# starlingonearth/MASt3R-SLAM-Quality-dualTSDF

Hardware: AMD Instinct MI355X
Metric: SLAM frames/sec (infer+match+TSDF+GN) @512x384 (higher is better)
Workload: dtype bf16

## Files before the change

### include/mslam_hip.h

```cpp
#ifndef MSLAM_HIP_H
#define MSLAM_HIP_H

#include <stddef.h>
#include <stdint.h>

#ifdef __cplusplus
extern "C" {
#endif

#define MSLAM_OK 0
#define MSLAM_EINVAL (-1)
#define MSLAM_EHIP (-2)
#define MSLAM_ENOMEM (-3)
#define MSLAM_ENODEV (-4)

const char* mslam_last_error(void);
int mslam_abi_version(void);
int mslam_device_check(void);


int mslam_iter_proj(const float* rays_img_with_grad, const float* pts_3d_norm,
                    const float* p_init, float* p_new, uint8_t* converged, int b, int h, int w,
                    int n, int max_iter, float lambda_init, float cost_thresh, void* stream);

// ... 39 lines not shown
int mslam_gn_compact(const float* Xs, const float* Cs, const int64_t* idx_ii2jj, const uint8_t* valid_match,
                     const float* Q, int num_poses, int num_points, int num_edges, int edge_begin,
                     int edge_count, float C_thresh, float Q_thresh, void* workspace, size_t workspace_bytes,
                     void* stream);
int mslam_gn_compact_at(const float* Xs, const float* Cs, const int64_t* idx_ii2jj, const uint8_t* valid_match,
                        const float* Q, int num_poses, int num_points, int num_edges, int edge_begin, int edge_count,
                        int slot_begin, int range_count, float C_thresh, float Q_thresh, void* workspace,
                        size_t workspace_bytes, void* stream);
int mslam_gn_accumulate(int kind, const float* Twc, const float* K, int num_poses, int num_points,
                        int num_edges, int edge_begin, int edge_count, float sigma_a, float sigma_b,
                        int height, int width, int pixel_border, float z_eps, float* Hs, float* gs,
                        void* workspace, size_t workspace_bytes, void* stream);
int mslam_gn_solve_retract(const float* Hs, const float* gs, int num_poses, int num_edges,
                           int num_points, float* Twc, float* dx, float delta_thresh, void* workspace,
                           size_t workspace_bytes, void* stream);
int mslam_gn_status(int* status4, int num_poses, int num_edges, int num_points, void* workspace,
                    size_t workspace_bytes, void* stream);

int mslam_sim3_act(const float* T, const float* X, float* Y, int num_poses, long long pts_per_pose,
                   int broadcast_pose, void* stream);
int mslam_sim3_op(int op, const float* A, const float* B, float* out, int n, int bcast_a, int bcast_b,
                  void* stream);

size_t mslam_tsdf_table_bytes(uint64_t capacity);
int mslam_tsdf_table_init(void* table, size_t table_bytes, uint64_t capacity, void* stream);

size_t mslam_tsdf_integrate_workspace_bytes(int n_points, double voxel_size, double trunc, double step_scale);
int mslam_tsdf_integrate(void* table, uint64_t capacity, const float* points_world, const double* conf,
                         const float* cam_origin, int n_points, double voxel_size, double trunc,
                         double max_weight, double step_scale, int shard_id, int num_shards,
// ... 244 lines not shown
```

### mast3r-slam-quality-dualtsdf_amd/csrc/gn.hip

```cpp
#include "common.h"
#include "sim3.h"

namespace mslam {

constexpr int kAcc = 35;
constexpr int kEdgeConst = 16;
constexpr int kPlanes = 8;
constexpr int kTile = 64;

struct GnState {
  int done;
  int iters;
  int chol_fail;
  float last_norm;
};

__device__ __forceinline__ int64_t ij_val(const int64_t* ii, const int64_t* jj, int E, int k) {
  return k < E ? ii[k] : jj[k - E];
}

__global__ __launch_bounds__(256) void gn_first_kernel(const int64_t* __restrict__ ii,
                                                       const int64_t* __restrict__ jj, int E,
                                                       int* __restrict__ first) {
  const int k = blockIdx.x * 256 + threadIdx.x;
// ... 25 lines not shown
  if (st->done) return;
  const int e = blockIdx.x * blockDim.x + threadIdx.x;
  if (e >= E) return;
  const Sim3f Ti = sim3_load(Twc + 8 * ii_edge[e]);
  const Sim3f Tj = sim3_load(Twc + 8 * jj_edge[e]);
  const Sim3f Tij = sim3_rel(Ti, Tj);
  float R[9];
  quat_to_mat(Tij.q, R);
  float* c = econst + (size_t)e * kEdgeConst;
#pragma unroll
  for (int k = 0; k < 9; k++) c[k] = Tij.s * R[k];
  c[9] = Tij.t[0]; c[10] = Tij.t[1]; c[11] = Tij.t[2];
  c[12] = c[13] = c[14] = c[15] = 0.0f;
}

__global__ __launch_bounds__(256) void gn_compact_kernel(
    const float* __restrict__ Xs, const float* __restrict__ Cs, const int* __restrict__ ii_edge,
    const int* __restrict__ jj_edge, const int64_t* __restrict__ idx_ii2jj,
    const uint8_t* __restrict__ valid_match, const float* __restrict__ Q, int num_points, int chunk_len,
    float C_thresh, float Q_thresh, float* __restrict__ stream, int* __restrict__ counts, int S, int slot_begin) {
  const int e = blockIdx.x / S, chunk = blockIdx.x - e * S;
  const int ix = ii_edge[e], jx = jj_edge[e];
  const float* __restrict__ Xi_base = Xs + (size_t)ix * num_points * 3;
  const float* __restrict__ Xj_base = Xs + (size_t)jx * num_points * 3;
  const float* __restrict__ Ci_base = Cs + (size_t)ix * num_points;
  const float* __restrict__ Cj_base = Cs + (size_t)jx * num_points;
  const int64_t* __restrict__ idx_e = idx_ii2jj + (size_t)e * num_points;
  const uint8_t* __restrict__ vm_e = valid_match + (size_t)e * num_points;
  const float* __restrict__ Q_e = Q + (size_t)e * num_points;
  float* __restrict__ slot = stream + ((size_t)(slot_begin + e) * S + chunk) * (size_t)chunk_len * kPlanes;
  __shared__ int wave_cnt[4];
  const int lane = threadIdx.x & 63, wid = threadIdx.x >> 6;
  const int k_begin = chunk * chunk_len;
  const int k_end = min(k_begin + chunk_len, num_points);
  int base = 0;
  for (int k0 = k_begin; k0 < k_end; k0 += 256) {
    const int k = k0 + (int)threadIdx.x;
    bool valid = false;
    long long ind = 0;
    float q = 0.0f;
    if (k < k_end) {
      const bool vm = vm_e[k] != 0;
      ind = vm ? idx_e[k] : 0;
      q = Q_e[k];
      const float ci = Ci_base[ind], cj = Cj_base[k];
      valid = vm & (q > Q_thresh) & (ci > C_thresh) & (cj > C_thresh);
    }
    const unsigned long long m = __ballot(valid);
    if (lane == 0) wave_cnt[wid] = __popcll(m);
    __syncthreads();
    int off = base;
    for (int w = 0; w < wid; w++) off += wave_cnt[w];
    const int total = wave_cnt[0] + wave_cnt[1] + wave_cnt[2] + wave_cnt[3];
    if (valid) {
      const int pos = off + __popcll(m & ((1ull << lane) - 1ull));
      slot[0 * (size_t)chunk_len + pos] = Xi_base[ind * 3 + 0];
      slot[1 * (size_t)chunk_len + pos] = Xi_base[ind * 3 + 1];
      slot[2 * (size_t)chunk_len + pos] = Xi_base[ind * 3 + 2];
      slot[3 * (size_t)chunk_len + pos] = Xj_base[(size_t)k * 3 + 0];
      slot[4 * (size_t)chunk_len + pos] = Xj_base[(size_t)k * 3 + 1];
      slot[5 * (size_t)chunk_len + pos] = Xj_base[(size_t)k * 3 + 2];
      slot[6 * (size_t)chunk_len + pos] = sqrtf(q);
      slot[7 * (size_t)chunk_len + pos] = __int_as_float((int)ind);
    }
    base += total;
    __syncthreads();
  }
  if (threadIdx.x == 0) counts[(slot_begin + e) * S + chunk] = base;
}

__device__ __forceinline__ float fast_rcp(float x) { return __builtin_amdgcn_rcpf(x); }
__device__ __forceinline__ float fast_rsq(float x) { return __builtin_amdgcn_rsqf(x); }

__device__ __forceinline__ float huber_w(float r) {
  return fminf(1.0f, 1.345f * fast_rcp(fabsf(r)));
}

template <unsigned NZ>
__device__ __forceinline__ void accum_row(float (&acc)[kAcc], const float (&x)[7], float w, float err) {
  const float we = w * err;
  int l = 0;
#pragma unroll
  for (int n = 0; n < 7; n++) {
// ... 100 lines not shown
    {
      const float x[7] = {1.0f, 0.0f, 0.0f, 0.0f, p2, -p1, p0};
      accum_row<0b1110001>(acc, x, w0, e0);
    }
    {
      const float x[7] = {0.0f, 1.0f, 0.0f, -p2, 0.0f, p0, p1};
      accum_row<0b1101010>(acc, x, w1, e1);
    }
    {
      const float x[7] = {0.0f, 0.0f, 1.0f, p1, -p0, 0.0f, p2};
      accum_row<0b1011100>(acc, x, w2, e2);
    }
  }
}

template <int KIND>
__global__ __launch_bounds__(256) void gn_accum_kernel(const GnState* __restrict__ st,
                                                       const float* __restrict__ econst,
                                                       const float* __restrict__ stream,
                                                       const int* __restrict__ counts, int chunk_len,
                                                       GnParams P, float* __restrict__ partial, int S) {
  if (st->done) return;
  const int e = blockIdx.x / S, chunk = blockIdx.x - e * S;
  const float* cc = econst + (size_t)e * kEdgeConst;
  const EdgeConst c = {cc[0], cc[1], cc[2], cc[3], cc[4], cc[5], cc[6], cc[7], cc[8], cc[9], cc[10], cc[11]};
  const float* __restrict__ slot = stream + ((size_t)e * S + chunk) * (size_t)chunk_len * kPlanes;
  const int n = counts[e * S + chunk];

  float acc[kAcc];
#pragma unroll
  for (int l = 0; l < kAcc; l++) acc[l] = 0.0f;

  const int n4 = n & ~3;
  for (int k = (int)threadIdx.x * 4; k < n4; k += 1024) {
    float f[kPlanes][4];
#pragma unroll
    for (int p = 0; p < kPlanes; p++) {
      if (p < (KIND == 1 ? 8 : 7)) {
        const float4 v = *reinterpret_cast<const float4*>(slot + (size_t)p * chunk_len + k);
        f[p][0] = v.x; f[p][1] = v.y; f[p][2] = v.z; f[p][3] = v.w;
      } else {
        f[p][0] = f[p][1] = f[p][2] = f[p][3] = 0.0f;
// ... 558 lines not shown
  float* econst;
  float* Hs;
  float* gs;
  double* Haug;
  double* Ldiag;
  double* xs;
  int* tmin32;
  int* counts;
  float* partial;
  float* stream;
  int S, chunk_len, np, ld, nb;
  size_t bytes_fixed;
  size_t bytes;
};

static GnWorkspace gn_carve(void* base, int P, int E, int HW, int local_edges) {
  GnWorkspace w;
  const int N = P > 1 ? P - 1 : 0;
  const int n = N * 7;
  w.np = (int)align_up((size_t)(n > 0 ? n : 1), kTile);
  w.ld = w.np;
  w.nb = 32;
  int S = E > 0 ? (1024 + E - 1) / E : 1;
  const int s_cap = HW / (256 * 16) > 0 ? HW / (256 * 16) : 1;
  if (S > s_cap) S = s_cap;
  if (S < 1) S = 1;
  w.S = S;
  w.chunk_len = (int)align_up((size_t)((HW + S - 1) / S), 256);
  if (w.chunk_len < 256) w.chunk_len = 256;
  size_t off = 0;
  auto take = [&](size_t bytes) { size_t o = off; off = align_up(off + bytes, 256); return (char*)base + o; };
  w.st = (GnState*)take(sizeof(GnState));
  w.ii_edge = (int*)take(sizeof(int) * (size_t)E);
  w.jj_edge = (int*)take(sizeof(int) * (size_t)E);
  w.ii_opt = (int*)take(sizeof(int) * (size_t)E);
  w.jj_opt = (int*)take(sizeof(int) * (size_t)E);
  w.first = (int*)take(sizeof(int) * 2 * (size_t)E);
  w.econst = (float*)take(sizeof(float) * (size_t)E * kEdgeConst);
  w.Hs = (float*)take(sizeof(float) * (size_t)4 * E * 49);
  w.gs = (float*)take(sizeof(float) * (size_t)2 * E * 7);
  w.Haug = (double*)take(sizeof(double) * (size_t)(w.np + 1) * w.ld);
  w.Ldiag = (double*)take(sizeof(double) * (size_t)w.np * w.nb);
  w.xs = (double*)take(sizeof(double) * (size_t)w.np);
  w.tmin32 = (int*)take(sizeof(int) * (size_t)(w.np / 32 + 2));
  w.bytes_fixed = off;
  const size_t L = local_edges > 0 ? (size_t)local_edges : 0;
  w.counts = (int*)take(sizeof(int) * L * S);
  w.partial = (float*)take(sizeof(float) * L * S * kAcc);
  w.stream = (float*)take(sizeof(float) * L * S * (size_t)w.chunk_len * kPlanes);
  w.bytes = off;
  return w;
}

static void fill_params(GnParams& P, int kind, const float* K_dev, float sigma_a, float sigma_b, int height,
                        int width, int pixel_border, float z_eps) {
  P.sa_inv = 1.0f / sigma_a;
  P.sb_inv = kind == 2 ? 0.0f : 1.0f / sigma_b;
  P.C_thresh = 0.0f;
  P.Q_thresh = 0.0f;
  P.height = height;
  P.width = width > 0 ? width : 1;
  P.border_lo = (float)pixel_border;
  P.border_hi_u = (float)(width - 1 - pixel_border);
  P.border_hi_v = (float)(height - 1 - pixel_border);
  P.z_eps = z_eps;
  P.K = K_dev;
}

static int launch_accumulate(int kind, const GnWorkspace& w, const float* Twc, int E, int e0, int cnt,
                             const GnParams& P, float* Hs, float* gs, hipStream_t s) {
  if (cnt <= 0) return MSLAM_OK;
  hipLaunchKernelGGL(gn_edge_setup_kernel, dim3((cnt + 63) / 64), dim3(64), 0, s, w.st, Twc, w.ii_edge + e0,
                     w.jj_edge + e0, cnt, w.econst);
  dim3 grid((unsigned)w.S * (unsigned)cnt);
  if (kind == 0)
    hipLaunchKernelGGL(gn_accum_kernel<0>, grid, dim3(256), 0, s, w.st, w.econst, w.stream, w.counts, w.chunk_len,
                       P, w.partial, w.S);
  else if (kind == 1)
    hipLaunchKernelGGL(gn_accum_kernel<1>, grid, dim3(256), 0, s, w.st, w.econst, w.stream, w.counts, w.chunk_len,
                       P, w.partial, w.S);
  else
    hipLaunchKernelGGL(gn_accum_kernel<2>, grid, dim3(256), 0, s, w.st, w.econst, w.stream, w.counts, w.chunk_len,
                       P, w.partial, w.S);
  hipLaunchKernelGGL(gn_reduce_kernel, dim3(cnt), dim3(64), 0, s, w.st, w.partial, w.S, Twc, w.ii_edge + e0, e0, E,
                     Hs, gs);
  return check_hip(hipGetLastError(), "gn accumulate launch");
}

template <int NB>
static int launch_cholesky(const GnWorkspace& w, hipStream_t s) {
  constexpr size_t shmem = sizeof(double) * (2 * kTile * (NB + 2) + NB * (NB + 1) + 2 * NB);
  static bool attr_set = false;
  if (shmem > 48 * 1024 && !attr_set) {
    int rc = check_hip(hipFuncSetAttribute((const void*)chol_step_kernel<NB>,
                                           hipFuncAttributeMaxDynamicSharedMemorySize, (int)shmem),
                       "hipFuncSetAttribute(chol_step)");
    if (rc) return rc;
    attr_set = true;
// ... 83 lines not shown
                                   const uint8_t* valid_match, const float* Q, int num_poses, int num_points,
                                   int num_edges, int edge_begin, int edge_count, int slot_begin, int range_count,
                                   float C_thresh, float Q_thresh, void* workspace, size_t workspace_bytes,
                                   void* stream) {
  MSLAM_REQUIRE(num_poses >= 2 && num_points >= 1 && num_edges >= 1, "gn_compact: bad sizes");
  MSLAM_REQUIRE(edge_begin >= 0 && edge_count >= 0 && edge_begin + edge_count <= num_edges,
                "gn_compact: edge range [%d,%d) outside [0,%d)", edge_begin, edge_begin + edge_count, num_edges);
  MSLAM_REQUIRE(slot_begin >= 0 && slot_begin + edge_count <= range_count,
                "gn_compact: slots [%d,%d) outside the accumulate range of %d edges", slot_begin,
                slot_begin + edge_count, range_count);
  if (edge_count == 0) return MSLAM_OK;
  MSLAM_REQUIRE(Xs && Cs && idx_ii2jj && valid_match && Q, "gn_compact: null pointer");
  GnWorkspace w = gn_carve(workspace, num_poses, num_edges, num_points, range_count);
  int rc = gn_check_ws(w.bytes, workspace, workspace_bytes, "gn_compact");
  if (rc) return rc;
  hipLaunchKernelGGL(gn_compact_kernel, dim3((unsigned)w.S * (unsigned)edge_count), dim3(256), 0, (hipStream_t)stream, Xs,
                     Cs, w.ii_edge + edge_begin, w.jj_edge + edge_begin, idx_ii2jj, valid_match, Q, num_points,
                     w.chunk_len, C_thresh, Q_thresh, w.stream, w.counts, w.S, slot_begin);
  return check_hip(hipGetLastError(), "gn_compact launch");
}

extern "C" int mslam_gn_compact(const float* Xs, const float* Cs, const int64_t* idx_ii2jj,
                                const uint8_t* valid_match, const float* Q, int num_poses, int num_points,
                                int num_edges, int edge_begin, int edge_count, float C_thresh, float Q_thresh,
                                void* workspace, size_t workspace_bytes, void* stream) {
  return mslam_gn_compact_at(Xs, Cs, idx_ii2jj, valid_match, Q, num_poses, num_points, num_edges, edge_begin,
                             edge_count, 0, edge_count, C_thresh, Q_thresh, workspace, workspace_bytes, stream);
}

extern "C" int mslam_gn_accumulate(int kind, const float* Twc, const float* K, int num_poses, int num_points,
                                   int num_edges, int edge_begin, int edge_count, float sigma_a, float sigma_b,
                                   int height, int width, int pixel_border, float z_eps, float* Hs, float* gs,
                                   void* workspace, size_t workspace_bytes, void* stream) {
  MSLAM_REQUIRE(kind >= 0 && kind <= 2, "gn_accumulate: kind must be 0 (rays), 1 (calib) or 2 (points)");
// ... 153 lines not shown
```

### mast3r-slam-quality-dualtsdf_amd/mast3r_slam/config.py

```python
import copy

_BASE = {
    "use_calib": False,
    "single_thread": False,
    "dataset": {"subsample": 1, "img_downsample": 1, "center_principle_point": True},
    "matching": {
        "max_iter": 10, "lambda_init": 1e-8, "convergence_thresh": 1e-6, "dist_thresh": 1e-1,
        "radius": 3, "dilation_max": 5,
    },
    "tracking": {
        "min_match_frac": 0.05, "max_iters": 50, "C_conf": 0.0, "Q_conf": 1.5, "rel_error": 1e-3,
        "delta_norm": 1e-3, "huber": 1.345, "match_frac_thresh": 0.333, "sigma_ray": 0.003,
        "sigma_dist": 1e1, "sigma_pixel": 1.0, "sigma_depth": 1e1, "sigma_point": 0.05,
        "pixel_border": -10, "depth_eps": 1e-6, "filtering_mode": "weighted_pointmap",
        "filtering_score": "median",
    },
    "local_opt": {
        "pin": 1, "window_size": 1e6, "C_conf": 0.0, "Q_conf": 1.5, "min_match_frac": 0.1,
        "pixel_border": -10, "depth_eps": 1e-6, "max_iters": 10, "sigma_ray": 0.003, "sigma_dist": 1e1,
        "sigma_pixel": 1.0, "sigma_depth": 1e1, "sigma_point": 0.05, "delta_norm": 1e-8, "use_cuda": True,
    },
    "retrieval": {"k": 3, "min_thresh": 5e-3},
    "reloc": {"min_match_frac": 0.3, "strict": True},
    "tsdf_refine": {
        "enabled": True, "window_size": 5, "voxel_size": 0.02, "trunc_dist": 0.08, "max_grid_dim": 64,
        "roi_size": 0.4, "ray_samples": 64, "max_displacement": 0.015, "min_weight_threshold": 0.01,
        "confidence_boost": 0.08, "confidence_max": 1.3, "min_hit_rate": 0.05, "max_rois_per_kf": 3,
        "min_confidence": 0.2, "pose_stable_thresh": 0.01,
    },
    "tsdf_global": {
        "enabled": False, "voxel_size": 0.03, "trunc_dist": 0.12, "max_weight": 100.0,
        "min_tsdf_weight": 1.0e-3, "max_points_per_kf": 40000, "min_confidence": 0.05,
        "samples_per_kf": 2000, "lambda": 0.15, "max_iterations": 3, "pre_icp_iters": 2, "damping": 1.0e-4,
        "color": False,
        "mesh_min_component_faces": 0,
# ... 27 lines not shown
```

### mast3r-slam-quality-dualtsdf_amd/mast3r_slam/global_opt.py

```python
import threading

import torch

import mast3r_slam_backends
import mslam_hip as _m
from lietorch_hip import Sim3
from mast3r_slam.config import config
from mast3r_slam.geometry import constrain_points_to_ray
from mast3r_slam.mast3r_utils import mast3r_match_symmetric


class FactorGraph:
    def __init__(self, model, frames, K=None, device="cuda", shard_edges=False, channel=None):
        self.model = model
        self.frames = frames
        self.device = device
        self.cfg = config["local_opt"]
        self._rows = {k: _Rows(dt, self.device) for k, dt in (
            ("ii", torch.long), ("jj", torch.long), ("idx_ii2jj", torch.long), ("idx_jj2ii", torch.long),
            ("valid_match_j", torch.bool), ("valid_match_i", torch.bool), ("Q_ii2jj", torch.float32),
            ("Q_jj2ii", torch.float32))}
        self.window_size = self.cfg["window_size"]
        self.K = K
        self.last_unique_kf_idx = None
        self.shard_edges = shard_edges
        self.reuse_tracking_decode = True
        self.reused_rows = 0
        self.channel = channel
        self.group = channel.group if channel is not None else None
        self._sent_tokens = {}
        self._sent_stamp = {}
        self.lock = threading.Lock()
        self._pm_cache = None

    def add_factors(self, ii, jj, min_match_frac, is_reloc=False):
        kf_ii = [self.frames[idx] for idx in ii]
        kf_jj = [self.frames[idx] for idx in jj]
        feat_i = torch.cat([kf.feat for kf in kf_ii])
        feat_j = torch.cat([kf.feat for kf in kf_jj])
        pos_i = torch.cat([kf.pos for kf in kf_ii])
        pos_j = torch.cat([kf.pos for kf in kf_jj])
        shape_i = [kf.img_true_shape for kf in kf_ii]
        shape_j = [kf.img_true_shape for kf in kf_jj]
        if self._driver:
            self._announce_add_factors(ii, jj, min_match_frac, is_reloc)
        if self.shard_edges and torch.distributed.is_available() and torch.distributed.is_initialized():
            res = match_symmetric_sharded(self.model, feat_i, pos_i, feat_j, pos_j, shape_i, shape_j, group=self.group)
        else:
# ... 70 lines not shown
        invalid = (~(ii_t == (jj_t - 1))) & invalid
        keep = (~invalid).cpu().tolist()
        if is_reloc and not all(keep):
            return False
        if all(keep):
            sel = lambda t: t
        else:
            rows_kept = torch.tensor([r for r, k in enumerate(keep) if k], dtype=torch.long, device=ii_t.device)
            sel = lambda t: t.index_select(0, rows_kept)
        picked = [("ii", sel(ii_t)), ("jj", sel(jj_t)), ("idx_ii2jj", sel(idx_i2j)), ("idx_jj2ii", sel(idx_j2i)),
                  ("valid_match_j", sel(valid_match_j)), ("valid_match_i", sel(valid_match_i)),
                  ("Q_ii2jj", sel(Qj)), ("Q_jj2ii", sel(Qi))]
        with self.lock:
            for name, rows in picked:
                self._rows[name].append(rows)
        return any(keep)

    ii = property(lambda self: self._rows["ii"].view)
    jj = property(lambda self: self._rows["jj"].view)
    idx_ii2jj = property(lambda self: self._rows["idx_ii2jj"].view)
    idx_jj2ii = property(lambda self: self._rows["idx_jj2ii"].view)
    valid_match_j = property(lambda self: self._rows["valid_match_j"].view)
    valid_match_i = property(lambda self: self._rows["valid_match_i"].view)
    Q_ii2jj = property(lambda self: self._rows["Q_ii2jj"].view)
    Q_jj2ii = property(lambda self: self._rows["Q_jj2ii"].view)

    @property
    def n_edges(self):
        return self._rows["ii"].n

    def two_way_sources(self, n_edges=None):
# ... 42 lines not shown
                c["keys"][r] = key
                if kf.X_canon.is_cuda:
                    cur = torch.cuda.current_stream(dev)
                    kf.X_canon.record_stream(cur)
                    kf.C.record_stream(cur)
        T_WCs = Sim3(torch.stack([kf.T_WC.data for kf in kfs]))
        return c["X"][:P], T_WCs, c["C"][:P]

    def prepare_solve(self, kind, n_edges=None):
        pin = self.cfg["pin"]
        with self.lock:
            if n_edges is not None:
                n_edges = min(int(n_edges), self.n_edges)
            unique_kf_idx = self.get_unique_kf_idx(n_edges)
            ii, jj, sources = self.two_way_sources(n_edges)
        if unique_kf_idx.numel() <= pin:
            self.last_unique_kf_idx = None
            return None
        if ii.is_cuda:
            cur = torch.cuda.current_stream(ii.device)
            for blk in sources:
                for t in blk:
                    t.record_stream(cur)
        self.last_unique_kf_idx = unique_kf_idx.detach().cpu()
        if hasattr(self.frames, "stamp"):
            Xs, T_WCs, Cs = self._poses_points_cached(self.last_unique_kf_idx.tolist())
        else:
            Xs, T_WCs, Cs = self.get_poses_points(unique_kf_idx)
        K = self.K
        height = width = 0
        if kind == "calib":
            img_size = self.frames[0].img.shape[-2:]
            Xs = constrain_points_to_ray(img_size, Xs, K)
            height, width = int(img_size[0]), int(img_size[1])
        job = dict(kind=kind, pin=pin, unique_kf_idx=unique_kf_idx, unique_kf_idx_host=self.last_unique_kf_idx, K=K,
                   height=height, width=width,
                   pose_data=T_WCs.data[:, 0, :].contiguous(), Xs=Xs.contiguous(), Cs=Cs.contiguous(),
                   edges=(ii, jj, sources))
        if self._driver:
            stamp = getattr(self.frames, "stamp", None)
            dirty = []
            for r, k in enumerate(self.last_unique_kf_idx.tolist()):
                st = stamp(k) if stamp is not None else None
                if st is None or self._sent_stamp.get(k) != st:
                    dirty.append((r, int(k)))
                    self._sent_stamp[k] = st
            job["dirty"] = dirty
        return job

    def run_solve(self, job):
        c, kind, K = self.cfg, job["kind"], job["K"]
        pose_data, Xs, Cs = job["pose_data"], job["Xs"], job["Cs"]
        ii, jj, sources = job["edges"]
        if self._driver:
            self._announce_solve(job)
        sharded = self.shard_edges and torch.distributed.is_available() and torch.distributed.is_initialized()
        gauss_newton_split(kind, pose_data, Xs, Cs, K, ii, jj, sources, c, job["height"], job["width"],
                           group=self.group, sharded=sharded)
        job["Xs"] = job["Cs"] = job["edges"] = None

    def commit_solve(self, job):
        pin = job["pin"]
        self.frames.update_T_WCs(Sim3(job["pose_data"][:, None, :])[pin:], job["unique_kf_idx_host"][pin:])

    def _solve(self, kind):
        job = self.prepare_solve(kind)
        if job is not None:
            self.run_solve(job)
            self.commit_solve(job)

    def solve_GN_rays(self):
        self._solve("rays")

    def solve_GN_calib(self):
# ... 43 lines not shown
            dist.broadcast(t, src=src, group=group)


def edge_slice(E, rank, world):
    base, rem = divmod(E, world)
    begin = rank * base + min(rank, rem)
    return begin, base + (1 if rank < rem else 0)


def gauss_newton_sharded(kind, Twc, Xs, Cs, K, ii, jj, idx_ii2jj, valid_match, Q, cfg, height=0, width=0,
                         group=None):
    return gauss_newton_split(kind, Twc, Xs, Cs, K, ii, jj, [(idx_ii2jj, valid_match, Q)], cfg, height, width,
                              group=group, sharded=True)


def gauss_newton_split(kind, Twc, Xs, Cs, K, ii, jj, sources, cfg, height=0, width=0, group=None, sharded=False):
    rank, world = 0, 1
    if sharded:
        import torch.distributed as dist

        rank, world = dist.get_rank(group), dist.get_world_size(group)
    P, HW, E = Xs.shape[0], Xs.shape[1], ii.shape[0]
    e0, cnt = edge_slice(E, rank, world)
    dev = Twc.device
    L = _m.lib()
    ws = mast3r_slam_backends._workspace(L.mslam_gn_workspace_bytes(P, E, HW, cnt), dev)
    blocks = torch.zeros(4 * E * 49 + 2 * E * 7, dtype=torch.float32, device=dev)
    Hs, gs = blocks[: 4 * E * 49], blocks[4 * E * 49:]
    dx = torch.zeros((P - 1, 7), dtype=torch.float32, device=dev)
    kid = {"rays": 0, "calib": 1, "points": 2}[kind]
    sa, sb = {"rays": (cfg["sigma_ray"], cfg["sigma_dist"]), "calib": (cfg["sigma_pixel"], cfg["sigma_depth"]),
              "points": (cfg.get("sigma_point", 0.05), 1.0)}[kind]
    _m.check(L.mslam_gn_begin(_m.ptr(ii), _m.ptr(jj), P, E, HW, _m.ptr(ws), ws.numel(), _m.stream_ptr()), "gn_begin")
    keep, b0 = [], 0
    for idx_b, vm_b, Q_b in sources:
        nb = idx_b.shape[0]
        lo, hi = max(e0, b0), min(e0 + cnt, b0 + nb)
        if hi > lo:
            idx_l, vm_l, Q_l = (t[lo - b0:hi - b0].contiguous() for t in (idx_b, vm_b, Q_b))
            keep.append((idx_l, vm_l, Q_l))
            rc = L.mslam_gn_compact_at(_m.ptr(Xs), _m.ptr(Cs), _m.ptr(idx_l), _m.ptr(vm_l), _m.ptr(Q_l), P, HW, E, lo,
                                       hi - lo, lo - e0, cnt, float(cfg["C_conf"]), float(cfg["Q_conf"]), _m.ptr(ws),
                                       ws.numel(), _m.stream_ptr())
            _m.check(rc, "gn_compact_at")
        b0 += nb
    assert b0 == E, (b0, E)
    for _ in range(int(cfg["max_iters"])):
        blocks.zero_()
        rc = L.mslam_gn_accumulate(
            kid, _m.ptr(Twc), _m.ptr(K) if K is not None else 0, P, HW, E, e0, cnt, float(sa), float(sb),
            int(height), int(width), int(cfg["pixel_border"]), float(cfg["depth_eps"]), _m.ptr(Hs), _m.ptr(gs),
            _m.ptr(ws), ws.numel(), _m.stream_ptr())
        _m.check(rc, "gn_accumulate")
        if world > 1:
            dist.all_reduce(blocks, op=dist.ReduceOp.SUM, group=group)
        rc = L.mslam_gn_solve_retract(_m.ptr(Hs), _m.ptr(gs), P, E, HW, _m.ptr(Twc), _m.ptr(dx),
                                      float(cfg["delta_norm"]), _m.ptr(ws), ws.numel(), _m.stream_ptr())
        _m.check(rc, "gn_solve_retract")
    return dx


class _Rows:

    def __init__(self, dtype, device):
        self.dtype, self.device, self.buf, self.n = dtype, device, None, 0

    def append(self, rows):
        k = int(rows.shape[0])
        if k == 0:
            return
        if self.buf is None or tuple(self.buf.shape[1:]) != tuple(rows.shape[1:]):
            assert self.n == 0, "row shape changed"
            self.buf = torch.empty((max(8, k),) + tuple(rows.shape[1:]), dtype=self.dtype, device=rows.device)
        if self.n + k > self.buf.shape[0]:
# ... 13 lines not shown
```

### mast3r-slam-quality-dualtsdf_amd/mast3r_slam/slam_system.py

```python
import contextlib
import os
import queue
import threading
import time

import torch

from lietorch_hip import Sim3
from mast3r_slam import mast3r_utils as mu
from mast3r_slam.config import config
from mast3r_slam.frame import KeyframeStore, Mode
from mast3r_slam.global_opt import FactorGraph
from mast3r_slam.tracker import FrameTracker


class RecentKeyframes:

    def __init__(self, keyframes, k=1):
        self.keyframes, self.k = keyframes, k

    def update(self, frame, add_after_query=True, k=3, min_thresh=0.0):
        if add_after_query:
            return []
        n = len(self.keyframes)
# ... 94 lines not shown
                                       next_stage=post, priority=solve_priority)
                self._worker = _BackendThread(self, lambda idx, _: self._backend_graph(idx), next_stage=solve,
                                              priority=self.backend_priority)
            else:
                self._worker = _BackendThread(self, lambda idx, _: self._backend(idx), priority=self.backend_priority)
        self.mode = Mode.INIT
        self.last_T = None
        self.frame_group = max(1, int(frame_group))
        self.encoder_group = self.frame_group if encoder_group is None else max(1, int(encoder_group))
        self.enc_stream = torch.cuda.Stream(device=self.device, priority=int(encoder_priority)) if self.frame_group > 1 else None
        self._enc_hi = 0
        self._kf_value, self._kf_slope = None, None
        self._n_pending = 0
        self.decode_ahead = max(0, int(decode_ahead)) if self.frame_group > 1 else 0
        self.dec_stream = torch.cuda.Stream(device=self.device) if self.decode_ahead > 0 else None
        self.stats = dict(frames=0, keyframes=0, group_calls=0, decoded_rows=0, void_rows=0, relocalised=0)

    def run(self, frames, start=0, stop=None, release=False):
        out = []
        stop = len(frames) if stop is None else min(stop, len(frames))
        self._enc_hi = max(self._enc_hi, start)
        if not self.pipeline:
            for i in range(start, stop):
                if self.frame_group > 1:
                    self._look_ahead(frames, i, stop)
                out.append(self.step(frames[i]))
                if release:
                    frames[i] = None
            return out
        i, pend = start, []
        while i < stop or pend:
# ... 627 lines not shown
```

Baseline: 164.6.

## Cache compacted GN correspondence streams across solves in a persistent slot store

Adds a persistent device-side store of compacted per-edge correspondence streams, keyed by edge stamps, so Gauss-Newton solves only re-run compaction for edges whose inputs changed and read the rest from cached slots. The accumulate kernel gains a store mode that looks up each edge's slot and falls back to workspace for overflow edges. The compact kernel also processes four rounds per iteration to overlap gathers. This costs extra GPU memory (up to a configurable cap) and depends on the stamps correctly invalidating stale edges.

```diff
diff --git a/include/mslam_hip.h b/include/mslam_hip.h
--- a/include/mslam_hip.h
+++ b/include/mslam_hip.h
@@ -77,6 +77,16 @@
 int mslam_gn_solve_retract(const float* Hs, const float* gs, int num_poses, int num_edges,
                            int num_points, float* Twc, float* dx, float delta_thresh, void* workspace,
                            size_t workspace_bytes, void* stream);
+size_t mslam_gn_store_workspace_bytes(int num_poses, int num_edges, int num_points, int fallback_edges);
+int mslam_gn_store_layout(int num_edges, int num_points, int* S, int* chunk_len, size_t* slot_bytes);
+int mslam_gn_store_compact(const float* Xs, const float* Cs, const int64_t* idx_ii2jj, const uint8_t* valid_match,
+                           const float* Q, int num_poses, int num_points, int num_edges, int edge_begin, int edge_count,
+                           const int* pairs, int num_pairs, float C_thresh, float Q_thresh, void* store,
+                           size_t store_bytes, int fallback_edges, void* workspace, size_t workspace_bytes, void* stream);
+int mslam_gn_store_accumulate(int kind, const float* Twc, const float* K, int num_poses, int num_points, int num_edges,
+                              float sigma_a, float sigma_b, int height, int width, int pixel_border, float z_eps,
+                              float* Hs, float* gs, const int* slot_of_edge, const void* store, size_t store_bytes,
+                              int fallback_edges, void* workspace, size_t workspace_bytes, void* stream);
 int mslam_gn_status(int* status4, int num_poses, int num_edges, int num_points, void* workspace,
                     size_t workspace_bytes, void* stream);
 
diff --git a/mast3r-slam-quality-dualtsdf_amd/csrc/gn.hip b/mast3r-slam-quality-dualtsdf_amd/csrc/gn.hip
--- a/mast3r-slam-quality-dualtsdf_amd/csrc/gn.hip
+++ b/mast3r-slam-quality-dualtsdf_amd/csrc/gn.hip
@@ -63,12 +63,46 @@
   c[12] = c[13] = c[14] = c[15] = 0.0f;
 }
 
+struct GnStore {
+  size_t slot_bytes;
+  int slots;
+  int ws_slots;
+};
+
+__device__ __forceinline__ size_t store_counts_offset(int S, int chunk_len) {
+  return sizeof(float) * (size_t)S * (size_t)chunk_len * kPlanes;
+}
+
+template <bool STORE>
 __global__ __launch_bounds__(256) void gn_compact_kernel(
     const float* __restrict__ Xs, const float* __restrict__ Cs, const int* __restrict__ ii_edge,
     const int* __restrict__ jj_edge, const int64_t* __restrict__ idx_ii2jj,
     const uint8_t* __restrict__ valid_match, const float* __restrict__ Q, int num_points, int chunk_len,
-    float C_thresh, float Q_thresh, float* __restrict__ stream, int* __restrict__ counts, int S, int slot_begin) {
-  const int e = blockIdx.x / S, chunk = blockIdx.x - e * S;
+    float C_thresh, float Q_thresh, float* __restrict__ stream, int* __restrict__ counts, int S, int slot_begin,
+    const int* __restrict__ pairs, int edge_count, char* __restrict__ store_base, GnStore store) {
+  const int b = blockIdx.x / S, chunk = blockIdx.x - b * S;
+  int e = b;
+  float* __restrict__ slot;
+  int* __restrict__ count_out;
+  if constexpr (STORE) {
+    e = pairs[2 * b];
+    const int s = pairs[2 * b + 1];
+    if (e < 0 || e >= edge_count) return;
+    if (s >= 0) {
+      if (s >= store.slots) return;
+      char* rec = store_base + (size_t)s * store.slot_bytes;
+      slot = reinterpret_cast<float*>(rec) + (size_t)chunk * (size_t)chunk_len * kPlanes;
+      count_out = reinterpret_cast<int*>(rec + store_counts_offset(S, chunk_len)) + chunk;
+    } else {
+      const int k = -(s + 1);
+      if (k >= store.ws_slots) return;
+      slot = stream + ((size_t)k * S + chunk) * (size_t)chunk_len * kPlanes;
+      count_out = counts + (size_t)k * S + chunk;
+    }
+  } else {
+    slot = stream + ((size_t)(slot_begin + e) * S + chunk) * (size_t)chunk_len * kPlanes;
+    count_out = counts + (slot_begin + e) * S + chunk;
+  }
   const int ix = ii_edge[e], jx = jj_edge[e];
   const float* __restrict__ Xi_base = Xs + (size_t)ix * num_points * 3;
   const float* __restrict__ Xj_base = Xs + (size_t)jx * num_points * 3;
@@ -77,45 +111,74 @@
   const int64_t* __restrict__ idx_e = idx_ii2jj + (size_t)e * num_points;
   const uint8_t* __restrict__ vm_e = valid_match + (size_t)e * num_points;
   const float* __restrict__ Q_e = Q + (size_t)e * num_points;
-  float* __restrict__ slot = stream + ((size_t)(slot_begin + e) * S + chunk) * (size_t)chunk_len * kPlanes;
-  __shared__ int wave_cnt[4];
+  constexpr int kRounds = 4;
+  __shared__ int wave_cnt[kRounds][4];
   const int lane = threadIdx.x & 63, wid = threadIdx.x >> 6;
   const int k_begin = chunk * chunk_len;
   const int k_end = min(k_begin + chunk_len, num_points);
   int base = 0;
-  for (int k0 = k_begin; k0 < k_end; k0 += 256) {
-    const int k = k0 + (int)threadIdx.x;
-    bool valid = false;
-    long long ind = 0;
-    float q = 0.0f;
-    if (k < k_end) {
-      const bool vm = vm_e[k] != 0;
-      ind = vm ? idx_e[k] : 0;
-      q = Q_e[k];
-      const float ci = Ci_base[ind], cj = Cj_base[k];
-      valid = vm & (q > Q_thresh) & (ci > C_thresh) & (cj > C_thresh);
-    }
-    const unsigned long long m = __ballot(valid);
-    if (lane == 0) wave_cnt[wid] = __popcll(m);
+  for (int k0 = k_begin; k0 < k_end; k0 += 256 * kRounds) {
+    bool vm[kRounds];
+    long long ind[kRounds];
+    float q[kRounds], cj[kRounds], ci[kRounds];
+    unsigned long long m[kRounds];
+#pragma unroll
+    for (int r = 0; r < kRounds; r++) {
+      const int k = k0 + r * 256 + (int)threadIdx.x;
+      vm[r] = false;
+      ind[r] = 0;
+      q[r] = cj[r] = 0.0f;
+      if (k < k_end) {
+        vm[r] = vm_e[k] != 0;
+        ind[r] = vm[r] ? idx_e[k] : 0;
+        q[r] = Q_e[k];
+        cj[r] = Cj_base[k];
+      }
+    }
+#pragma unroll
+    for (int r = 0; r < kRounds; r++) ci[r] = (k0 + r * 256 + (int)threadIdx.x < k_end) ? Ci_base[ind[r]] : 0.0f;
+#pragma unroll
+    for (int r = 0; r < kRounds; r++) {
+      const bool in_range = k0 + r * 256 + (int)threadIdx.x < k_end;
+      const bool valid = in_range & vm[r] & (q[r] > Q_thresh) & (ci[r] > C_thresh) & (cj[r] > C_thresh);
+      vm[r] = valid;
+      m[r] = __ballot(valid);
+      if (lane == 0) wave_cnt[r][wid] = __popcll(m[r]);
+    }
     __syncthreads();
-    int off = base;
-    for (int w = 0; w < wid; w++) off += wave_cnt[w];
-    const int total = wave_cnt[0] + wave_cnt[1] + wave_cnt[2] + wave_cnt[3];
-    if (valid) {
-      const int pos = off + __popcll(m & ((1ull << lane) - 1ull));
-      slot[0 * (size_t)chunk_len + pos] = Xi_base[ind * 3 + 0];
-      slot[1 * (size_t)chunk_len + pos] = Xi_base[ind * 3 + 1];
-      slot[2 * (size_t)chunk_len + pos] = Xi_base[ind * 3 + 2];
-      slot[3 * (size_t)chunk_len + pos] = Xj_base[(size_t)k * 3 + 0];
-      slot[4 * (size_t)chunk_len + pos] = Xj_base[(size_t)k * 3 + 1];
-      slot[5 * (size_t)chunk_len + pos] = Xj_base[(size_t)k * 3 + 2];
-      slot[6 * (size_t)chunk_len + pos] = sqrtf(q);
-      slot[7 * (size_t)chunk_len + pos] = __int_as_float((int)ind);
-    }
-    base += total;
+    float xi[kRounds][3], xj[kRounds][3];
+    int pos[kRounds];
+#pragma unroll
+    for (int r = 0; r < kRounds; r++) {
+      int off = base;
+      for (int w = 0; w < wid; w++) off += wave_cnt[r][w];
+      base += wave_cnt[r][0] + wave_cnt[r][1] + wave_cnt[r][2] + wave_cnt[r][3];
+      pos[r] = off + __popcll(m[r] & ((1ull << lane) - 1ull));
+      if (vm[r]) {
+        const size_t k = (size_t)(k0 + r * 256 + (int)threadIdx.x);
+#pragma unroll
+        for (int a = 0; a < 3; a++) {
+          xi[r][a] = Xi_base[ind[r] * 3 + a];
+          xj[r][a] = Xj_base[k * 3 + a];
+        }
+      }
+    }
+#pragma unroll
+    for (int r = 0; r < kRounds; r++) {
+      if (vm[r]) {
+        slot[0 * (size_t)chunk_len + pos[r]] = xi[r][0];
+        slot[1 * (size_t)chunk_len + pos[r]] = xi[r][1];
+        slot[2 * (size_t)chunk_len + pos[r]] = xi[r][2];
+        slot[3 * (size_t)chunk_len + pos[r]] = xj[r][0];
+        slot[4 * (size_t)chunk_len + pos[r]] = xj[r][1];
+        slot[5 * (size_t)chunk_len + pos[r]] = xj[r][2];
+        slot[6 * (size_t)chunk_len + pos[r]] = sqrtf(q[r]);
+        slot[7 * (size_t)chunk_len + pos[r]] = __int_as_float((int)ind[r]);
+      }
+    }
     __syncthreads();
   }
-  if (threadIdx.x == 0) counts[(slot_begin + e) * S + chunk] = base;
+  if (threadIdx.x == 0) *count_out = base;
 }
 
 __device__ __forceinline__ float fast_rcp(float x) { return __builtin_amdgcn_rcpf(x); }
@@ -246,18 +309,36 @@
   }
 }
 
-template <int KIND>
+template <int KIND, bool STORE>
 __global__ __launch_bounds__(256) void gn_accum_kernel(const GnState* __restrict__ st,
                                                        const float* __restrict__ econst,
                                                        const float* __restrict__ stream,
                                                        const int* __restrict__ counts, int chunk_len,
-                                                       GnParams P, float* __restrict__ partial, int S) {
+                                                       GnParams P, float* __restrict__ partial, int S,
+                                                       const int* __restrict__ slot_of_edge,
+                                                       const char* __restrict__ store_base, GnStore store) {
   if (st->done) return;
   const int e = blockIdx.x / S, chunk = blockIdx.x - e * S;
   const float* cc = econst + (size_t)e * kEdgeConst;
   const EdgeConst c = {cc[0], cc[1], cc[2], cc[3], cc[4], cc[5], cc[6], cc[7], cc[8], cc[9], cc[10], cc[11]};
   const float* __restrict__ slot = stream + ((size_t)e * S + chunk) * (size_t)chunk_len * kPlanes;
-  const int n = counts[e * S + chunk];
+  int n;
+  if constexpr (STORE) {
+    const int s = __builtin_amdgcn_readfirstlane(slot_of_edge[e]);
+    const bool in_store = s >= 0;
+    const int k = in_store ? s : -(s + 1);
+    const char* rec = store_base + (size_t)k * store.slot_bytes;
+    const float* first = in_store ? reinterpret_cast<const float*>(rec) : stream + (size_t)k * S * (size_t)chunk_len * kPlanes;
+    const int* cnt = in_store ? reinterpret_cast<const int*>(rec + store_counts_offset(S, chunk_len)) : counts + (size_t)k * S;
+    slot = first + (size_t)chunk * (size_t)chunk_len * kPlanes;
+    n = 0;
+    if (k < (in_store ? store.slots : store.ws_slots)) n = cnt[chunk];
+    n = min(n, chunk_len);
+    if (n < 0) n = 0;
+    n = __builtin_amdgcn_readfirstlane(n);
+  } else {
+    n = counts[e * S + chunk];
+  }
 
   float acc[kAcc];
 #pragma unroll
@@ -846,7 +927,7 @@
   size_t bytes;
 };
 
-static GnWorkspace gn_carve(void* base, int P, int E, int HW, int local_edges) {
+static GnWorkspace gn_carve(void* base, int P, int E, int HW, int local_edges, int stream_edges = -1) {
   GnWorkspace w;
   const int N = P > 1 ? P - 1 : 0;
   const int n = N * 7;
@@ -877,9 +958,10 @@
   w.tmin32 = (int*)take(sizeof(int) * (size_t)(w.np / 32 + 2));
   w.bytes_fixed = off;
   const size_t L = local_edges > 0 ? (size_t)local_edges : 0;
-  w.counts = (int*)take(sizeof(int) * L * S);
+  const size_t Ls = stream_edges >= 0 ? (size_t)stream_edges : L;
+  w.counts = (int*)take(sizeof(int) * Ls * S);
   w.partial = (float*)take(sizeof(float) * L * S * kAcc);
-  w.stream = (float*)take(sizeof(float) * L * S * (size_t)w.chunk_len * kPlanes);
+  w.stream = (float*)take(sizeof(float) * Ls * S * (size_t)w.chunk_len * kPlanes);
   w.bytes = off;
   return w;
 }
@@ -899,21 +981,32 @@
   P.K = K_dev;
 }
 
+template <bool STORE>
+static void launch_accum_kernel(int kind, const GnWorkspace& w, dim3 grid, const GnParams& P, const int* slot_of_edge,
+                                const char* store_base, const GnStore& store, hipStream_t s) {
+  if (kind == 0)
+    hipLaunchKernelGGL((gn_accum_kernel<0, STORE>), grid, dim3(256), 0, s, w.st, w.econst, w.stream, w.counts,
+                       w.chunk_len, P, w.partial, w.S, slot_of_edge, store_base, store);
+  else if (kind == 1)
+    hipLaunchKernelGGL((gn_accum_kernel<1, STORE>), grid, dim3(256), 0, s, w.st, w.econst, w.stream, w.counts,
+                       w.chunk_len, P, w.partial, w.S, slot_of_edge, store_base, store);
+  else
+    hipLaunchKernelGGL((gn_accum_kernel<2, STORE>), grid, dim3(256), 0, s, w.st, w.econst, w.stream, w.counts,
+                       w.chunk_len, P, w.partial, w.S, slot_of_edge, store_base, store);
+}
+
 static int launch_accumulate(int kind, const GnWorkspace& w, const float* Twc, int E, int e0, int cnt,
-                             const GnParams& P, float* Hs, float* gs, hipStream_t s) {
+                             const GnParams& P, float* Hs, float* gs, hipStream_t s,
+                             const int* slot_of_edge = nullptr, const char* store_base = nullptr,
+                             const GnStore& store = GnStore{0, 0, 0}) {
   if (cnt <= 0) return MSLAM_OK;
   hipLaunchKernelGGL(gn_edge_setup_kernel, dim3((cnt + 63) / 64), dim3(64), 0, s, w.st, Twc, w.ii_edge + e0,
                      w.jj_edge + e0, cnt, w.econst);
   dim3 grid((unsigned)w.S * (unsigned)cnt);
-  if (kind == 0)
-    hipLaunchKernelGGL(gn_accum_kernel<0>, grid, dim3(256), 0, s, w.st, w.econst, w.stream, w.counts, w.chunk_len,
-                       P, w.partial, w.S);
-  else if (kind == 1)
-    hipLaunchKernelGGL(gn_accum_kernel<1>, grid, dim3(256), 0, s, w.st, w.econst, w.stream, w.counts, w.chunk_len,
-                       P, w.partial, w.S);
+  if (slot_of_edge)
+    launch_accum_kernel<true>(kind, w, grid, P, slot_of_edge, store_base, store, s);
   else
-    hipLaunchKernelGGL(gn_accum_kernel<2>, grid, dim3(256), 0, s, w.st, w.econst, w.stream, w.counts, w.chunk_len,
-                       P, w.partial, w.S);
+    launch_accum_kernel<false>(kind, w, grid, P, nullptr, nullptr, store, s);
   hipLaunchKernelGGL(gn_reduce_kernel, dim3(cnt), dim3(64), 0, s, w.st, w.partial, w.S, Twc, w.ii_edge + e0, e0, E,
                      Hs, gs);
   return check_hip(hipGetLastError(), "gn accumulate launch");
@@ -1027,10 +1120,82 @@
   GnWorkspace w = gn_carve(workspace, num_poses, num_edges, num_points, range_count);
   int rc = gn_check_ws(w.bytes, workspace, workspace_bytes, "gn_compact");
   if (rc) return rc;
-  hipLaunchKernelGGL(gn_compact_kernel, dim3((unsigned)w.S * (unsigned)edge_count), dim3(256), 0, (hipStream_t)stream, Xs,
-                     Cs, w.ii_edge + edge_begin, w.jj_edge + edge_begin, idx_ii2jj, valid_match, Q, num_points,
-                     w.chunk_len, C_thresh, Q_thresh, w.stream, w.counts, w.S, slot_begin);
+  hipLaunchKernelGGL(gn_compact_kernel<false>, dim3((unsigned)w.S * (unsigned)edge_count), dim3(256), 0,
+                     (hipStream_t)stream, Xs, Cs, w.ii_edge + edge_begin, w.jj_edge + edge_begin, idx_ii2jj, valid_match, Q,
+                     num_points, w.chunk_len, C_thresh, Q_thresh, w.stream, w.counts, w.S, slot_begin, nullptr, edge_count,
+                     nullptr, GnStore{0, 0, 0});
   return check_hip(hipGetLastError(), "gn_compact launch");
+}
+
+static size_t gn_store_slot_bytes(const GnWorkspace& w) {
+  return sizeof(float) * (size_t)w.S * (size_t)w.chunk_len * kPlanes + align_up(sizeof(int) * (size_t)w.S, 256);
+}
+
+static GnStore gn_store_view(const GnWorkspace& w, const void* store, size_t store_bytes, int fallback_edges) {
+  GnStore v;
+  v.slot_bytes = gn_store_slot_bytes(w);
+  const size_t slots = store ? store_bytes / v.slot_bytes : 0;
+  v.slots = (int)(slots < (size_t)0x7fffffff ? slots : (size_t)0x7fffffff);
+  v.ws_slots = fallback_edges;
+  return v;
+}
+
+extern "C" size_t mslam_gn_store_workspace_bytes(int num_poses, int num_edges, int num_points, int fallback_edges) {
+  if (num_poses < 0 || num_edges < 0 || num_points < 0 || fallback_edges < 0 || fallback_edges > num_edges) return 0;
+  return gn_carve(nullptr, num_poses, num_edges, num_points, num_edges, fallback_edges).bytes;
+}
+
+extern "C" int mslam_gn_store_layout(int num_edges, int num_points, int* S, int* chunk_len, size_t* slot_bytes) {
+  MSLAM_REQUIRE(num_edges >= 1 && num_points >= 1, "gn_store_layout: bad sizes");
+  MSLAM_REQUIRE(S && chunk_len && slot_bytes, "gn_store_layout: null pointer");
+  GnWorkspace w = gn_carve(nullptr, 2, num_edges, num_points, 0);
+  *S = w.S;
+  *chunk_len = w.chunk_len;
+  *slot_bytes = gn_store_slot_bytes(w);
+  return MSLAM_OK;
+}
+
+extern "C" int mslam_gn_store_compact(const float* Xs, const float* Cs, const int64_t* idx_ii2jj,
+                                      const uint8_t* valid_match, const float* Q, int num_poses, int num_points,
+                                      int num_edges, int edge_begin, int edge_count, const int* pairs, int num_pairs,
+                                      float C_thresh, float Q_thresh, void* store, size_t store_bytes,
+                                      int fallback_edges, void* workspace, size_t workspace_bytes, void* stream) {
+  MSLAM_REQUIRE(num_poses >= 2 && num_points >= 1 && num_edges >= 1, "gn_store_compact: bad sizes");
+  MSLAM_REQUIRE(edge_begin >= 0 && edge_count >= 0 && edge_begin + edge_count <= num_edges,
+                "gn_store_compact: edge range [%d,%d) outside [0,%d)", edge_begin, edge_begin + edge_count, num_edges);
+  MSLAM_REQUIRE(num_pairs >= 0 && fallback_edges >= 0 && fallback_edges <= num_edges,
+                "gn_store_compact: %d pairs, %d fallback edges of %d", num_pairs, fallback_edges, num_edges);
+  if (num_pairs == 0) return MSLAM_OK;
+  MSLAM_REQUIRE(Xs && Cs && idx_ii2jj && valid_match && Q && pairs, "gn_store_compact: null pointer");
+  GnWorkspace w = gn_carve(workspace, num_poses, num_edges, num_points, num_edges, fallback_edges);
+  int rc = gn_check_ws(w.bytes, workspace, workspace_bytes, "gn_store_compact");
+  if (rc) return rc;
+  MSLAM_REQUIRE((unsigned long long)w.S * (unsigned long long)num_pairs <= 0x7fffffffull, "gn_store_compact: grid too large");
+  hipLaunchKernelGGL(gn_compact_kernel<true>, dim3((unsigned)w.S * (unsigned)num_pairs), dim3(256), 0,
+                     (hipStream_t)stream, Xs, Cs, w.ii_edge + edge_begin, w.jj_edge + edge_begin, idx_ii2jj, valid_match, Q,
+                     num_points, w.chunk_len, C_thresh, Q_thresh, w.stream, w.counts, w.S, 0, pairs, edge_count,
+                     (char*)store, gn_store_view(w, store, store_bytes, fallback_edges));
+  return check_hip(hipGetLastError(), "gn_store_compact launch");
+}
+
+extern "C" int mslam_gn_store_accumulate(int kind, const float* Twc, const float* K, int num_poses, int num_points,
+                                         int num_edges, float sigma_a, float sigma_b, int height, int width,
+                                         int pixel_border, float z_eps, float* Hs, float* gs, const int* slot_of_edge,
+                                         const void* store, size_t store_bytes, int fallback_edges, void* workspace,
+                                         size_t workspace_bytes, void* stream) {
+  MSLAM_REQUIRE(kind >= 0 && kind <= 2, "gn_store_accumulate: kind must be 0 (rays), 1 (calib) or 2 (points)");
+  MSLAM_REQUIRE(num_poses >= 2 && num_points >= 1 && num_edges >= 1, "gn_store_accumulate: bad sizes");
+  MSLAM_REQUIRE(fallback_edges >= 0 && fallback_edges <= num_edges, "gn_store_accumulate: %d fallback edges of %d",
+                fallback_edges, num_edges);
+  MSLAM_REQUIRE(Twc && Hs && gs && slot_of_edge, "gn_store_accumulate: null pointer");
+  MSLAM_REQUIRE(kind != 1 || (K && width > 0 && height > 0), "gn_store_accumulate: calib needs K, height, width");
+  GnWorkspace w = gn_carve(workspace, num_poses, num_edges, num_points, num_edges, fallback_edges);
+  int rc = gn_check_ws(w.bytes, workspace, workspace_bytes, "gn_store_accumulate");
+  if (rc) return rc;
+  GnParams P;
+  fill_params(P, kind, K, sigma_a, sigma_b, height, width, pixel_border, z_eps);
+  return launch_accumulate(kind, w, Twc, num_edges, 0, num_edges, P, Hs, gs, (hipStream_t)stream, slot_of_edge,
+                           (const char*)store, gn_store_view(w, store, store_bytes, fallback_edges));
 }
 
 extern "C" int mslam_gn_compact(const float* Xs, const float* Cs, const int64_t* idx_ii2jj,
diff --git a/mast3r-slam-quality-dualtsdf_amd/mast3r_slam/config.py b/mast3r-slam-quality-dualtsdf_amd/mast3r_slam/config.py
--- a/mast3r-slam-quality-dualtsdf_amd/mast3r_slam/config.py
+++ b/mast3r-slam-quality-dualtsdf_amd/mast3r_slam/config.py
@@ -19,6 +19,7 @@
         "pin": 1, "window_size": 1e6, "C_conf": 0.0, "Q_conf": 1.5, "min_match_frac": 0.1,
         "pixel_border": -10, "depth_eps": 1e-6, "max_iters": 10, "sigma_ray": 0.003, "sigma_dist": 1e1,
         "sigma_pixel": 1.0, "sigma_depth": 1e1, "sigma_point": 0.05, "delta_norm": 1e-8, "use_cuda": True,
+        "stream_store": True, "stream_store_max_bytes": 8 << 30,
     },
     "retrieval": {"k": 3, "min_thresh": 5e-3},
     "reloc": {"min_match_frac": 0.3, "strict": True},
diff --git a/mast3r-slam-quality-dualtsdf_amd/mast3r_slam/global_opt.py b/mast3r-slam-quality-dualtsdf_amd/mast3r_slam/global_opt.py
--- a/mast3r-slam-quality-dualtsdf_amd/mast3r_slam/global_opt.py
+++ b/mast3r-slam-quality-dualtsdf_amd/mast3r_slam/global_opt.py
@@ -32,6 +32,10 @@
         self._sent_stamp = {}
         self.lock = threading.Lock()
         self._pm_cache = None
+        self._stream = _StreamStore()
+        self._edge_kf = []
+        self.stats = None
+        self.last_solve_edges = (0, 0)
 
     def add_factors(self, ii, jj, min_match_frac, is_reloc=False):
         kf_ii = [self.frames[idx] for idx in ii]
@@ -132,7 +136,24 @@
         with self.lock:
             for name, rows in picked:
                 self._rows[name].append(rows)
+            host = lambda v: v.tolist() if hasattr(v, "tolist") else list(v)
+            self._edge_kf += [(int(i), int(j)) for i, j, k in zip(host(ii), host(jj), keep) if k]
         return any(keep)
+
+    def invalidate_stream_store(self):
+        self._stream.invalidate()
+
+    def _edge_stamps(self, n_rows):
+        stamp = getattr(self.frames, "stamp", None)
+        if stamp is None or self.shard_edges or not self.cfg.get("stream_store", True):
+            return None
+        if len(self._edge_kf) != self.n_edges:
+            self._edge_kf = list(zip(self.ii.cpu().tolist(), self.jj.cpu().tolist()))
+        out = []
+        for i, j in self._edge_kf[:n_rows]:
+            si, sj = stamp(i), stamp(j)
+            out.append(None if si is None or sj is None else (si, sj))
+        return out
 
     ii = property(lambda self: self._rows["ii"].view)
     jj = property(lambda self: self._rows["jj"].view)
@@ -205,6 +226,8 @@
                 n_edges = min(int(n_edges), self.n_edges)
             unique_kf_idx = self.get_unique_kf_idx(n_edges)
             ii, jj, sources = self.two_way_sources(n_edges)
+            edge_stamps = self._edge_stamps(self.n_edges if n_edges is None else n_edges)
+            rows_ref = self._rows["ii"]
         if unique_kf_idx.numel() <= pin:
             self.last_unique_kf_idx = None
             return None
@@ -227,7 +250,7 @@
         job = dict(kind=kind, pin=pin, unique_kf_idx=unique_kf_idx, unique_kf_idx_host=self.last_unique_kf_idx, K=K,
                    height=height, width=width,
                    pose_data=T_WCs.data[:, 0, :].contiguous(), Xs=Xs.contiguous(), Cs=Cs.contiguous(),
-                   edges=(ii, jj, sources))
+                   edges=(ii, jj, sources), edge_stamps=edge_stamps, rows_ref=rows_ref)
         if self._driver:
             stamp = getattr(self.frames, "stamp", None)
             dirty = []
@@ -246,9 +269,23 @@
         if self._driver:
             self._announce_solve(job)
         sharded = self.shard_edges and torch.distributed.is_available() and torch.distributed.is_initialized()
-        gauss_newton_split(kind, pose_data, Xs, Cs, K, ii, jj, sources, c, job["height"], job["width"],
-                           group=self.group, sharded=sharded)
-        job["Xs"] = job["Cs"] = job["edges"] = None
+        stamps = job.get("edge_stamps")
+        plan = None
+        if stamps is not None and not sharded and len(sources) == 2 and len(stamps) == sources[0][0].shape[0]:
+            plan = self._stream.plan(job["rows_ref"], stamps, kind, ii.shape[0], Xs.shape[1], c, pose_data.device)
+        try:
+            gauss_newton_split(kind, pose_data, Xs, Cs, K, ii, jj, sources, c, job["height"], job["width"],
+                               group=self.group, sharded=sharded, store_plan=plan, out=job.get("out"))
+        except Exception:
+            self._stream.invalidate()
+            raise
+        E = int(ii.shape[0])
+        compacted = E if plan is None else plan["compacted"]
+        self.last_solve_edges = (compacted, E - compacted)
+        if self.stats is not None:
+            self.stats["gn_edges_compacted"] = self.stats.get("gn_edges_compacted", 0) + compacted
+            self.stats["gn_edges_reused"] = self.stats.get("gn_edges_reused", 0) + E - compacted
+        job["Xs"] = job["Cs"] = job["edges"] = job["rows_ref"] = None
 
     def commit_solve(self, job):
         pin = job["pin"]
@@ -322,8 +359,10 @@
                               group=group, sharded=True)
 
 
-def gauss_newton_split(kind, Twc, Xs, Cs, K, ii, jj, sources, cfg, height=0, width=0, group=None, sharded=False):
+def gauss_newton_split(kind, Twc, Xs, Cs, K, ii, jj, sources, cfg, height=0, width=0, group=None, sharded=False,
+                       store_plan=None, out=None):
     rank, world = 0, 1
+    assert store_plan is None or not sharded
     if sharded:
         import torch.distributed as dist
 
@@ -332,7 +371,12 @@
     e0, cnt = edge_slice(E, rank, world)
     dev = Twc.device
     L = _m.lib()
-    ws = mast3r_slam_backends._workspace(L.mslam_gn_workspace_bytes(P, E, HW, cnt), dev)
+    sp = store_plan
+    if sp is None:
+        ws = mast3r_slam_backends._workspace(L.mslam_gn_workspace_bytes(P, E, HW, cnt), dev)
+    else:
+        ws = mast3r_slam_backends._workspace(L.mslam_gn_store_workspace_bytes(P, E, HW, sp["fallback"]), dev)
+        st_ptr, st_bytes = (_m.ptr(sp["store"]), sp["store"].numel()) if sp["store"] is not None else (0, 0)
     blocks = torch.zeros(4 * E * 49 + 2 * E * 7, dtype=torch.float32, device=dev)
     Hs, gs = blocks[: 4 * E * 49], blocks[4 * E * 49:]
     dx = torch.zeros((P - 1, 7), dtype=torch.float32, device=dev)
@@ -341,10 +385,20 @@
               "points": (cfg.get("sigma_point", 0.05), 1.0)}[kind]
     _m.check(L.mslam_gn_begin(_m.ptr(ii), _m.ptr(jj), P, E, HW, _m.ptr(ws), ws.numel(), _m.stream_ptr()), "gn_begin")
     keep, b0 = [], 0
-    for idx_b, vm_b, Q_b in sources:
+    for blk, (idx_b, vm_b, Q_b) in enumerate(sources):
         nb = idx_b.shape[0]
         lo, hi = max(e0, b0), min(e0 + cnt, b0 + nb)
-        if hi > lo:
+        if sp is not None:
+            off, n_pairs = sp["pairs"][blk]
+            if n_pairs:
+                idx_l, vm_l, Q_l = (t.contiguous() for t in (idx_b, vm_b, Q_b))
+                keep.append((idx_l, vm_l, Q_l))
+                rc = L.mslam_gn_store_compact(_m.ptr(Xs), _m.ptr(Cs), _m.ptr(idx_l), _m.ptr(vm_l), _m.ptr(Q_l), P, HW, E,
+                                              b0, nb, _m.ptr(sp["table"][off:]), n_pairs, float(cfg["C_conf"]),
+                                              float(cfg["Q_conf"]), st_ptr, st_bytes, sp["fallback"], _m.ptr(ws),
+                                              ws.numel(), _m.stream_ptr())
+                _m.check(rc, "gn_store_compact")
+        elif hi > lo:
             idx_l, vm_l, Q_l = (t[lo - b0:hi - b0].contiguous() for t in (idx_b, vm_b, Q_b))
             keep.append((idx_l, vm_l, Q_l))
             rc = L.mslam_gn_compact_at(_m.ptr(Xs), _m.ptr(Cs), _m.ptr(idx_l), _m.ptr(vm_l), _m.ptr(Q_l), P, HW, E, lo,
@@ -355,17 +409,96 @@
     assert b0 == E, (b0, E)
     for _ in range(int(cfg["max_iters"])):
         blocks.zero_()
-        rc = L.mslam_gn_accumulate(
-            kid, _m.ptr(Twc), _m.ptr(K) if K is not None else 0, P, HW, E, e0, cnt, float(sa), float(sb),
-            int(height), int(width), int(cfg["pixel_border"]), float(cfg["depth_eps"]), _m.ptr(Hs), _m.ptr(gs),
-            _m.ptr(ws), ws.numel(), _m.stream_ptr())
+        if sp is None:
+            rc = L.mslam_gn_accumulate(
+                kid, _m.ptr(Twc), _m.ptr(K) if K is not None else 0, P, HW, E, e0, cnt, float(sa), float(sb),
+                int(height), int(width), int(cfg["pixel_border"]), float(cfg["depth_eps"]), _m.ptr(Hs), _m.ptr(gs),
+                _m.ptr(ws), ws.numel(), _m.stream_ptr())
+        else:
+            rc = L.mslam_gn_store_accumulate(
+                kid, _m.ptr(Twc), _m.ptr(K) if K is not None else 0, P, HW, E, float(sa), float(sb), int(height),
+                int(width), int(cfg["pixel_border"]), float(cfg["depth_eps"]), _m.ptr(Hs), _m.ptr(gs),
+                _m.ptr(sp["table"]), st_ptr, st_bytes, sp["fallback"], _m.ptr(ws), ws.numel(), _m.stream_ptr())
         _m.check(rc, "gn_accumulate")
         if world > 1:
             dist.all_reduce(blocks, op=dist.ReduceOp.SUM, group=group)
         rc = L.mslam_gn_solve_retract(_m.ptr(Hs), _m.ptr(gs), P, E, HW, _m.ptr(Twc), _m.ptr(dx),
                                       float(cfg["delta_norm"]), _m.ptr(ws), ws.numel(), _m.stream_ptr())
         _m.check(rc, "gn_solve_retract")
+    if out is not None:
+        out["Hs"], out["gs"] = Hs, gs
     return dx
+
+
+class _StreamStore:
+
+    MIN_SLOTS = 16
+
+    def __init__(self):
+        self.buf, self.key, self.slot_bytes = None, None, 0
+        self.stamps = []
+        self.rows_ref, self.rows_seen = None, 0
+        self.stream = None
+
+    def invalidate(self):
+        self.stamps = []
+
+    @property
+    def capacity(self):
+        return 0 if self.buf is None or not self.slot_bytes else self.buf.numel() // self.slot_bytes
+
+    def plan(self, rows_ref, edge_stamps, kind, E, HW, cfg, dev):
+        import ctypes
+
+        n = len(edge_stamps)
+        assert E == 2 * n, (E, n)
+        S, chunk_len, slot_bytes = ctypes.c_int(), ctypes.c_int(), ctypes.c_size_t()
+        _m.check(_m.lib().mslam_gn_store_layout(E, HW, ctypes.addressof(S), ctypes.addressof(chunk_len),
+                                                ctypes.addressof(slot_bytes)), "gn_store_layout")
+        key = (S.value, chunk_len.value, int(HW), float(cfg["C_conf"]), float(cfg["Q_conf"]), kind == "calib", str(dev))
+        if key != self.key or rows_ref is not self.rows_ref or rows_ref.n < self.rows_seen:
+            self.invalidate()
+            self.key, self.slot_bytes, self.rows_ref = key, slot_bytes.value, rows_ref
+            if self.buf is not None and self.buf.device != torch.device(dev):
+                self.buf, self.stream = None, None
+        self.rows_seen = rows_ref.n
+        cap_slots = int(cfg.get("stream_store_max_bytes", 8 << 30)) // self.slot_bytes
+        want = min(E, cap_slots)
+        if self.capacity < want:
+            slots = min(max(2 * self.capacity, want, self.MIN_SLOTS), cap_slots)
+            grown = torch.empty(slots * self.slot_bytes, dtype=torch.uint8, device=dev)
+            used = min(len(self.stamps), self.capacity) * self.slot_bytes
+            if used and any(s is not None for s in self.stamps):
+                grown[:used].copy_(self.buf[:used])
+            self.buf = grown
+        if self.buf is not None and self.buf.is_cuda:
+            cur = torch.cuda.current_stream(dev)
+            if self.stream is not None and self.stream != cur:
+                self.buf.record_stream(cur)
+            self.stream = cur
+        capacity = self.capacity
+        if len(self.stamps) < min(E, capacity):
+            self.stamps += [None] * (min(E, capacity) - len(self.stamps))
+        slot_of_edge, pairs, fallback = [0] * E, ([], []), 0
+        for d in (0, 1):
+            for r, st in enumerate(edge_stamps):
+                slot = 2 * r + d
+                if slot < capacity:
+                    if st is None or self.stamps[slot] != st:
+                        pairs[d].extend((r, slot))
+                        self.stamps[slot] = st
+                else:
+                    slot = -(fallback + 1)
+                    fallback += 1
+                    pairs[d].extend((r, slot))
+                slot_of_edge[d * n + r] = slot
+        host = torch.tensor(slot_of_edge + pairs[0] + pairs[1], dtype=torch.int32)
+        if torch.device(dev).type == "cuda":
+            host = host.pin_memory()
+        table = host.to(dev, non_blocking=True)
+        return dict(store=self.buf, table=table, fallback=fallback,
+                    pairs=[(E, len(pairs[0]) // 2), (E + len(pairs[0]), len(pairs[1]) // 2)],
+                    compacted=(len(pairs[0]) + len(pairs[1])) // 2)
 
 
 class _Rows:
diff --git a/mast3r-slam-quality-dualtsdf_amd/mast3r_slam/slam_system.py b/mast3r-slam-quality-dualtsdf_amd/mast3r_slam/slam_system.py
--- a/mast3r-slam-quality-dualtsdf_amd/mast3r_slam/slam_system.py
+++ b/mast3r-slam-quality-dualtsdf_amd/mast3r_slam/slam_system.py
@@ -132,7 +132,9 @@
         self._n_pending = 0
         self.decode_ahead = max(0, int(decode_ahead)) if self.frame_group > 1 else 0
         self.dec_stream = torch.cuda.Stream(device=self.device) if self.decode_ahead > 0 else None
-        self.stats = dict(frames=0, keyframes=0, group_calls=0, decoded_rows=0, void_rows=0, relocalised=0)
+        self.stats = dict(frames=0, keyframes=0, group_calls=0, decoded_rows=0, void_rows=0, relocalised=0,
+                          gn_edges_compacted=0, gn_edges_reused=0)
+        self.factor_graph.stats = self.stats
 
     def run(self, frames, start=0, stop=None, release=False):
         out = []
```

Result: faster. 168.1, median of 6 (+2.1%).
